# tangxyw/RecAlgorithm

Measured on NVIDIA H100. Metric: ctr_fwd_bwd_samples_per_sec, higher is better.
Workload: dtype f32

## Files before the change

### recalgorithm_b200/csrc/cin_bwd.cu

```cuda
#include <stdlib.h>

#include "tc_ptx.cuh"

namespace ctr {
namespace cinb {
using namespace ctr::tc;

__global__ void split_filter_native_kernel(const float* __restrict__ w, float* __restrict__ ws, int K, int H, int KRP, int HP) {
  const size_t total = (size_t)KRP * HP;
  for (size_t idx = (size_t)blockIdx.x * blockDim.x + threadIdx.x; idx < total; idx += (size_t)gridDim.x * blockDim.x) {
    const int row = (int)(idx / HP), n = (int)(idx % HP);
    float v = 0.f;
    if (row < K && n < H) v = __ldg(w + (size_t)row * H + n);
    store_split(ws, total, idx, v);
  }
}
__global__ void split_grad_kernel(const float* __restrict__ g, float* __restrict__ gs, size_t total) {
  for (size_t idx = (size_t)blockIdx.x * blockDim.x + threadIdx.x; idx < total; idx += (size_t)gridDim.x * blockDim.x)
    store_split(gs, total, idx, __ldg(g + idx));
}

constexpr int DX_IPS = 2;
constexpr int DX_N = DX_IPS * KB;
constexpr int DX_TILE = NWG * WG_M;

template <int SB, int NKB>
__global__ void __launch_bounds__(NTHREADS, 1)
cin_bwd_dx_tc_kernel(const __grid_constant__ CUtensorMap tmap_w, const float* __restrict__ x0,
                     const float* __restrict__ xk, const float* __restrict__ g, float* __restrict__ dx0,
                     float* __restrict__ dxk, int B, int m, int hk, int logD, int H, int KRP) {
  extern __shared__ __align__(1024) uint8_t smem_raw[];
  uint8_t* smem = align_1024(smem_raw);
  constexpr int HP = NKB * KB;
  constexpr int b_copy_bytes = NKB * DX_N * 128;
  constexpr int stage_bytes = 2 * b_copy_bytes;
  const uint32_t sbase = smem_u32(smem);
  Ring ring(sbase + SB * stage_bytes, SB);

  const int warp = warp_uniform(threadIdx.x >> 5), lane = threadIdx.x & 31;
  const int D = 1 << logD;
  const long long rows_total = (long long)B * D;
  const int num_tiles = (int)((rows_total + DX_TILE - 1) / DX_TILE);
  const int nsteps = (hk + DX_IPS - 1) / DX_IPS;

  ring.init();
  if (producer_role(warp, lane, [&] {
        for (int tile = blockIdx.x; tile < num_tiles; tile += gridDim.x) {
          for (int st = 0; st < nsteps; ++st) {
            const Ring::Slot slot = ring.acquire(stage_bytes);
            const uint32_t dst = sbase + slot.stage * stage_bytes;
            tma_load_4d(dst, &tmap_w, 0, st * DX_IPS * m, 0, 0, slot.full);
            tma_load_4d(dst + b_copy_bytes, &tmap_w, 0, KRP + st * DX_IPS * m, 0, 0, slot.full);
          }
        }
      }))
    return;

  const int wg = warp >> 2, w = warp & 3, gq = lane >> 2, t = lane & 3;
  for (int tile = blockIdx.x; tile < num_tiles; tile += gridDim.x) {
    const long long base = (long long)tile * DX_TILE + wg * WG_M;
    bool valid[2];
    int bb[2], dd[2];
    float x0v[2][8], dx0acc[2][8];
    uint32_t gh[HP / 8][4], gl[HP / 8][4];
#pragma unroll
    for (int rr = 0; rr < 2; ++rr) {
      const long long r = base + w * 16 + gq + 8 * rr;
      valid[rr] = r < rows_total;
      bb[rr] = valid[rr] ? (int)(r >> logD) : 0;
      dd[rr] = (int)(r & (D - 1));
#pragma unroll
      for (int q = 0; q < 8; ++q) {
        const int j = 8 * (q >> 1) + 2 * t + (q & 1);
        x0v[rr][q] = (valid[rr] && j < m) ? __ldg(x0 + ((size_t)bb[rr] * m + j) * D + dd[rr]) : 0.f;
        dx0acc[rr][q] = 0.f;
      }
    }
#pragma unroll
    for (int ks = 0; ks < HP / 8; ++ks) {
      float ga[4];
#pragma unroll
      for (int q = 0; q < 4; ++q) {
        const int rr = q & 1, n = 8 * ks + t + 4 * (q >> 1);
        ga[q] = (valid[rr] && n < H) ? __ldg(g + ((size_t)bb[rr] * H + n) * D + dd[rr]) : 0.f;
      }
      tf32_split(ga, gh[ks], gl[ks]);
    }
    auto load_xi = [&](int i0, float (&xi)[2][DX_IPS]) {
#pragma unroll
      for (int rr = 0; rr < 2; ++rr)
#pragma unroll
        for (int h = 0; h < DX_IPS; ++h)
          xi[rr][h] = (valid[rr] && i0 + h < hk) ? __ldg(xk + ((size_t)bb[rr] * hk + i0 + h) * D + dd[rr]) : 0.f;
    };
    float xi[2][DX_IPS];
    load_xi(0, xi);
    for (int st = 0; st < nsteps; ++st) {
      const int i0 = st * DX_IPS;
      const int s = ring.wait();
      const uint64_t bhi = gmma_desc_kmajor(sbase + s * stage_bytes, 128);
      const uint64_t blo = gmma_desc_kmajor(sbase + s * stage_bytes + b_copy_bytes, 128);
      float dz[DX_N / 2];
#pragma unroll
      for (int q = 0; q < DX_N / 2; ++q) dz[q] = 0.f;
      wgmma_fence();
#pragma unroll
      for (int ks = 0; ks < HP / 8; ++ks) {
        const uint64_t off = (uint64_t)((ks >> 2) * (DX_N * 128 / 16) + 2 * (ks & 3));
        mma_3xtf32<DX_N>(dz, gh[ks], gl[ks], bhi, blo, off, ks > 0 ? 1 : 0);
      }
      wgmma_commit();
      float xin[2][DX_IPS];
      load_xi(i0 + DX_IPS, xin);
      wgmma_wait<0>();
      ring.release(lane);
#pragma unroll
      for (int h = 0; h < DX_IPS; ++h) {
#pragma unroll
        for (int rr = 0; rr < 2; ++rr) {
          float p = 0.f;
#pragma unroll
          for (int q = 0; q < 8; ++q) {
            const float v = dz[4 * (4 * h + (q >> 1)) + 2 * rr + (q & 1)];
            p += v * x0v[rr][q];
            dx0acc[rr][q] += v * xi[rr][h];
          }
          p += __shfl_xor_sync(0xffffffffu, p, 1);
          p += __shfl_xor_sync(0xffffffffu, p, 2);
          if (t == 0 && valid[rr] && i0 + h < hk) dxk[((size_t)bb[rr] * hk + i0 + h) * D + dd[rr]] = p;
        }
      }
#pragma unroll
      for (int rr = 0; rr < 2; ++rr)
#pragma unroll
        for (int h = 0; h < DX_IPS; ++h) xi[rr][h] = xin[rr][h];
    }
#pragma unroll
    for (int rr = 0; rr < 2; ++rr) {
#pragma unroll
      for (int q = 0; q < 8; ++q) {
        const int j = 8 * (q >> 1) + 2 * t + (q & 1);
        if (valid[rr] && j < m) dx0[((size_t)bb[rr] * m + j) * D + dd[rr]] = dx0acc[rr][q];
      }
    }
  }
}

constexpr int DW_IPC = NWG * 2;

template <int N, int D>
__global__ void __launch_bounds__(NTHREADS, 1)
cin_bwd_dw_tc_kernel(const __grid_constant__ CUtensorMap tmap_g, const float* __restrict__ x0,
                     const float* __restrict__ xk, float* __restrict__ dw, int B, int m, int hk, int H,
                     int ngroups, int nslices, int chunk, int SB) {
  extern __shared__ __align__(1024) uint8_t smem_raw[];
  uint8_t* smem = align_1024(smem_raw);
  constexpr int row_bytes = D * 4;
  constexpr int b_copy_bytes = N * row_bytes;
  constexpr int stage_bytes = 2 * b_copy_bytes;
  const uint32_t sbase = smem_u32(smem);
  Ring ring(sbase + SB * stage_bytes, SB);

  const int warp = warp_uniform(threadIdx.x >> 5), lane = threadIdx.x & 31;
  const int group = blockIdx.x % ngroups;
  int b_beg, b_end;
  batch_slice(blockIdx.x / ngroups, nslices, B, b_beg, b_end);

  ring.init();
  if (producer_role(warp, lane, [&] {
        for (int b = b_beg; b < b_end; ++b) {
          const Ring::Slot slot = ring.acquire(stage_bytes);
          const uint32_t dst = sbase + slot.stage * stage_bytes;
          tma_load_3d(dst, &tmap_g, 0, 0, b, slot.full);
          tma_load_3d(dst + b_copy_bytes, &tmap_g, 0, 0, B + b, slot.full);
        }
      }))
    return;

  const int wg = warp >> 2, w = warp & 3, gq = lane >> 2, t = lane & 3;
  const int i = group * DW_IPC + wg * 2 + (w >> 1);
  const int j0 = (w & 1) * 16 + gq, j1 = j0 + 8;
  const bool live0 = i < hk && j0 < m, live1 = i < hk && j1 < m;
  float acc[N / 2], dacc[N / 2];
#pragma unroll
  for (int q = 0; q < N / 2; ++q) { acc[q] = 0.f; dacc[q] = 0.f; }
  auto form = [&](int b, uint32_t (&fh)[D / 8][4], uint32_t (&fl)[D / 8][4]) {
    float xa[D / 4], xb0[D / 4], xb1[D / 4];
#pragma unroll
    for (int q = 0; q < D / 4; ++q) {
      const int d = 8 * (q >> 1) + t + 4 * (q & 1);
      xa[q] = i < hk ? __ldg(xk + ((size_t)b * hk + i) * D + d) : 0.f;
      xb0[q] = live0 ? __ldg(x0 + ((size_t)b * m + j0) * D + d) : 0.f;
      xb1[q] = live1 ? __ldg(x0 + ((size_t)b * m + j1) * D + d) : 0.f;
    }
#pragma unroll
    for (int k = 0; k < D / 8; ++k) {
      const float a[4] = {xa[2 * k] * xb0[2 * k], xa[2 * k] * xb1[2 * k], xa[2 * k + 1] * xb0[2 * k + 1],
                          xa[2 * k + 1] * xb1[2 * k + 1]};
      tf32_split(a, fh[k], fl[k]);
    }
  };
  uint32_t ah[D / 8][4], al[D / 8][4];
  if (b_end > b_beg) form(b_beg, ah, al);
  for (int b = b_beg; b < b_end; ++b) {
    const bool chunk_start = chain_first(b - b_beg, chunk);
    const int s = ring.wait();
    const uint64_t bhi = gmma_desc_kmajor(sbase + s * stage_bytes, row_bytes);
    const uint64_t blo = gmma_desc_kmajor(sbase + s * stage_bytes + b_copy_bytes, row_bytes);
    wgmma_fence();
#pragma unroll
    for (int k = 0; k < D / 8; ++k) mma_3xtf32<N>(dacc, ah[k], al[k], bhi, blo, 2 * k, (chunk_start && k == 0) ? 0 : 1);
    wgmma_commit();
    uint32_t bh[D / 8][4], bl[D / 8][4];
    form(b + 1 < b_end ? b + 1 : b, bh, bl);
    wgmma_wait_keep(ah, al);
    ring.release(lane);
    if (chain_last(b - b_beg, b_end - b_beg, chunk)) chain_drain(acc, dacc);
#pragma unroll
    for (int k = 0; k < D / 8; ++k)
#pragma unroll
      for (int q = 0; q < 4; ++q) { ah[k][q] = bh[k][q]; al[k][q] = bl[k][q]; }
  }
  if (b_end > b_beg) {
#pragma unroll
    for (int c = 0; c < N / 8; ++c) {
#pragma unroll
      for (int e = 0; e < 2; ++e) {
        const int n = 8 * c + 2 * t + e;
        if (n < H) {
          if (live0) atomicAdd(dw + ((size_t)i * m + j0) * H + n, acc[4 * c + e]);
          if (live1) atomicAdd(dw + ((size_t)i * m + j1) * H + n, acc[4 * c + 2 + e]);
        }
      }
    }
  }
}

__global__ void __launch_bounds__(256)
cin_bwd_dx_kernel(const float* __restrict__ x0, const float* __restrict__ xk, const float* __restrict__ w,
                  const float* __restrict__ g, int B, int m, int hk, int D, int H, float* __restrict__ dx0,
                  float* __restrict__ dxk) {
  extern __shared__ __align__(16) float sm[];
  float* x0s = sm;
  float* xks = x0s + m * D;
  float* gs = xks + hk * D;
  float* dx0s = gs + H * D;
  float* dxks = dx0s + m * D;
  const int d = threadIdx.x % D, pl = threadIdx.x / D, pstep = blockDim.x / D;
  for (int b = blockIdx.x; b < B; b += gridDim.x) {
    __syncthreads();
    for (int i = threadIdx.x; i < m * D; i += blockDim.x) { x0s[i] = __ldg(x0 + (size_t)b * m * D + i); dx0s[i] = 0.f; }
    for (int i = threadIdx.x; i < hk * D; i += blockDim.x) { xks[i] = __ldg(xk + (size_t)b * hk * D + i); dxks[i] = 0.f; }
    for (int i = threadIdx.x; i < H * D; i += blockDim.x) gs[i] = __ldg(g + (size_t)b * H * D + i);
    __syncthreads();
    if (pl < pstep) {
      for (int p = pl; p < hk * m; p += pstep) {
        const float* wr = w + (size_t)p * H;
        float dz = 0.f;
        for (int n = 0; n < H; ++n) dz += gs[n * D + d] * __ldg(wr + n);
        const int i = p / m, j = p % m;
        atomicAdd(dxks + i * D + d, dz * x0s[j * D + d]);
        atomicAdd(dx0s + j * D + d, dz * xks[i * D + d]);
      }
    }
    __syncthreads();
    for (int i = threadIdx.x; i < m * D; i += blockDim.x) dx0[(size_t)b * m * D + i] = dx0s[i];
    for (int i = threadIdx.x; i < hk * D; i += blockDim.x) dxk[(size_t)b * hk * D + i] = dxks[i];
  }
}

constexpr int CIN_PC = 16;
__global__ void __launch_bounds__(256)
cin_bwd_dw_kernel(const float* __restrict__ x0, const float* __restrict__ xk, const float* __restrict__ g, int B, int m,
                  int hk, int D, int H, float* __restrict__ dw) {
  extern __shared__ __align__(16) float sm[];
  float* gs = sm;
  float* zs = gs + H * (D + 1);
  const int p0 = blockIdx.x * CIN_PC;
  const int K = hk * m;
  float acc[CIN_PC];
#pragma unroll
  for (int q = 0; q < CIN_PC; ++q) acc[q] = 0.f;
  for (int b = blockIdx.y; b < B; b += gridDim.y) {
    __syncthreads();
    for (int i = threadIdx.x; i < H * D; i += blockDim.x) gs[(i / D) * (D + 1) + i % D] = __ldg(g + (size_t)b * H * D + i);
    for (int i = threadIdx.x; i < CIN_PC * D; i += blockDim.x) {
      const int q = i / D, d = i % D, p = p0 + q;
      float z = 0.f;
      if (p < K) z = __ldg(xk + ((size_t)b * hk + p / m) * D + d) * __ldg(x0 + ((size_t)b * m + p % m) * D + d);
      zs[i] = z;
    }
    __syncthreads();
    for (int n = threadIdx.x; n < H; n += blockDim.x) {
      for (int d = 0; d < D; ++d) {
        const float gv = gs[n * (D + 1) + d];
#pragma unroll
        for (int q = 0; q < CIN_PC; ++q) acc[q] += zs[q * D + d] * gv;
      }
    }
  }
  const int n = threadIdx.x;
  if (n < H) {
#pragma unroll
    for (int q = 0; q < CIN_PC; ++q)
      if (p0 + q < K) atomicAdd(dw + (size_t)(p0 + q) * H + n, acc[q]);
  }
}

static bool tensor_path_ok(int64_t m, int64_t hk, int64_t D, int64_t H) {
  return m >= 1 && m <= 32 && hk >= 1 && H >= 1 && H <= 128 && (D == 8 || D == 16 || D == 32);
}

}
}

using namespace ctr;
using namespace ctr::cinb;

extern "C" int64_t ctr_cin_bwd_workspace_bytes(int64_t B, int64_t m, int64_t hk, int64_t D, int64_t H) {
  if (!tensor_path_ok(m, hk, D, H)) return 0;
  const int64_t HP = pad_to(H, 32), KRP = (hk + 2) * m + 32;
  return ((2 * KRP + m) * HP + 2 * B * H * D) * (int64_t)sizeof(float);
}

extern "C" int ctr_cin_bwd(const float* x0, const float* xk, const float* filter, const float* g_out, int64_t B,
                           int64_t m, int64_t hk, int64_t D, int64_t H, float* dx0, float* dxk, float* dfilter,
                           void* workspace, int64_t workspace_bytes, void* stream) {
  static const char* fn = "ctr_cin_bwd";
  CTR_REQUIRE(B >= 0 && m >= 1 && hk >= 1 && D >= 1 && H >= 1, "ctr_cin_bwd: bad sizes B=%lld m=%lld hk=%lld D=%lld H=%lld",
              (long long)B, (long long)m, (long long)hk, (long long)D, (long long)H);
  CTR_UNSUPPORTED(B * D > 0x7fffffffLL || hk * m > (1 << 24), "ctr_cin_bwd: problem too large");
  CTR_REQUIRE(x0 && xk && filter && g_out && dx0 && dxk && dfilter, "ctr_cin_bwd: null argument");
  CTR_UNSUPPORTED(D > 256 || H > 256, "ctr_cin_bwd: D=%lld H=%lld too large", (long long)D, (long long)H);
  cudaStream_t st = as_stream(stream);
  CTR_CUDA(cudaMemsetAsync(dfilter, 0, sizeof(float) * hk * m * H, st));
  if (B == 0) return CTR_OK;
  const int sms = sm_count();
  int rc;
  if (!tensor_path_ok(m, hk, D, H)) {
    const size_t smem_dx = sizeof(float) * (size_t)(2 * (m + hk) + H) * D;
    CTR_UNSUPPORTED(smem_dx > 200 * 1024, "ctr_cin_bwd: shared memory need %zu B too large", smem_dx);
    const int grid = capped_grid(B, (int64_t)sms * 4);
    rc = launch("ctr_cin_bwd(dx)", cin_bwd_dx_kernel, grid, 256, smem_dx, st, x0, xk, filter, g_out, (int)B, (int)m,
                (int)hk, (int)D, (int)H, dx0, dxk);
    if (rc) return rc;
    const size_t smem_dw = sizeof(float) * (size_t)(H * (D + 1) + CIN_PC * D);
    CTR_UNSUPPORTED(smem_dw > 200 * 1024, "ctr_cin_bwd: shared memory need %zu B too large", smem_dw);
    const int gx = (int)((hk * m + CIN_PC - 1) / CIN_PC);
    int gy = (int)((int64_t)sms * 4 / gx);
    if (gy < 1) gy = 1;
    if (gy > B) gy = (int)B;
    return launch("ctr_cin_bwd(dw)", cin_bwd_dw_kernel, dim3(gx, gy), 256, smem_dw, st, x0, xk, g_out, (int)B, (int)m,
                  (int)hk, (int)D, (int)H, dfilter);
  }
  rc = check_workspace(fn, "ctr_cin_bwd_workspace_bytes", workspace, workspace_bytes,
                       ctr_cin_bwd_workspace_bytes(B, m, hk, D, H));
  if (rc) return rc;
  const int HP = (int)pad_to(H, 32), KRP = (int)((hk + 2) * m + 32);
  const int NP = pad3(H);
  float* ws_w = static_cast<float*>(workspace);
  float* ws_g = ws_w + (size_t)(2 * KRP + m) * HP;
  rc = launch("ctr_cin_bwd(split filter)", split_filter_native_kernel, capped_grid(((size_t)KRP * HP + 255) / 256, 2048), 256, 0, st,
              filter, ws_w, (int)(hk * m), (int)H, KRP, HP);
  if (rc) return rc;
  const size_t tg = (size_t)B * H * D;
  rc = launch("ctr_cin_bwd(split grad)", split_grad_kernel, capped_grid((tg + 255) / 256, 4096), 256, 0, st, g_out, ws_g, tg);
  if (rc) return rc;
  int logD = 0;
  while ((1 << logD) < D) ++logD;
  {
    CUtensorMap tmap;
    const cuuint64_t gdim[4] = {32, (cuuint64_t)(2 * KRP), (cuuint64_t)DX_IPS, (cuuint64_t)(HP / 32)};
    const cuuint64_t gstr[3] = {(cuuint64_t)HP * sizeof(float), (cuuint64_t)m * HP * sizeof(float), 32 * sizeof(float)};
    const cuuint32_t box[4] = {32, 32, (cuuint32_t)DX_IPS, (cuuint32_t)(HP / 32)};
    rc = encode_tmap(fn, &tmap, 4, ws_w, gdim, gstr, box, CU_TENSOR_MAP_SWIZZLE_128B);
    if (rc) return rc;
    constexpr int SB = 3;
    const int nkb = HP / 32;
    const int smem = SB * 2 * nkb * DX_N * 128 + 8 * 2 * SB + 1024;
    const long long rows = (long long)B * D;
    const int tiles = (int)((rows + DX_TILE - 1) / DX_TILE);
    const int grid = capped_grid(tiles, sms);
    rc = with_const<1, 2, 3, 4>(nkb, [&](auto NKB) {
      return launch("ctr_cin_bwd(dx, wgmma)", cin_bwd_dx_tc_kernel<SB, NKB>, grid, NTHREADS, smem, st, tmap, x0, xk, g_out,
                    dx0, dxk, (int)B, (int)m, (int)hk, logD, (int)H, KRP);
    });
    if (rc) return rc;
  }
  CUtensorMap tmap;
  const cuuint64_t gdim[3] = {(cuuint64_t)D, (cuuint64_t)H, (cuuint64_t)(2 * B)};
  const cuuint64_t gstr[2] = {(cuuint64_t)D * sizeof(float), (cuuint64_t)H * D * sizeof(float)};
  const cuuint32_t box[3] = {(cuuint32_t)D, (cuuint32_t)NP, 1};
  const CUtensorMapSwizzle sw = D == 32 ? CU_TENSOR_MAP_SWIZZLE_128B : D == 16 ? CU_TENSOR_MAP_SWIZZLE_64B
                                                                               : CU_TENSOR_MAP_SWIZZLE_32B;
  rc = encode_tmap(fn, &tmap, 3, ws_g, gdim, gstr, box, sw);
  if (rc) return rc;
  const int stage_bytes = 2 * NP * (int)D * 4;
  int sb = (192 * 1024) / stage_bytes;
  if (sb > 8) sb = 8;
  const int smem = sb * stage_bytes + 8 * 2 * sb + 1024;
  const int ngroups = (int)((hk + DW_IPC - 1) / DW_IPC);
  const int nslices = batch_slices(sms, ngroups, B);
  const int grid = ngroups * nslices;
  const int chunk = (int)(256 / D);
  return with_const<32, 64, 128>(NP, [&](auto N) {
    return with_const<8, 16, 32>((int)D, [&](auto DD) {
      return launch("ctr_cin_bwd(dw, wgmma)", cin_bwd_dw_tc_kernel<N, DD>, grid, NTHREADS, smem, st, tmap, x0, xk,
                    dfilter, (int)B, (int)m, (int)hk, (int)H, ngroups, nslices, chunk, sb);
    });
  });
}
```

### recalgorithm_b200/csrc/tc_ptx.cuh

```cuda
#pragma once
#include <cuda.h>

#include "ctr_common.cuh"

namespace ctr {
namespace tc {

constexpr int WG_M = 64;
constexpr int KB = 32;
constexpr int NWG = 2;
constexpr int NTHREADS = (NWG + 1) * 128;

__device__ __forceinline__ uint32_t smem_u32(const void* p) { return (uint32_t)__cvta_generic_to_shared(p); }

__device__ __forceinline__ void mbar_init(uint32_t bar, uint32_t count) {
  asm volatile("mbarrier.init.shared::cta.b64 [%0], %1;" ::"r"(bar), "r"(count) : "memory");
}
__device__ __forceinline__ void mbar_arrive(uint32_t bar) {
  asm volatile("mbarrier.arrive.shared::cta.b64 _, [%0];" ::"r"(bar) : "memory");
}
__device__ __forceinline__ void mbar_expect_tx(uint32_t bar, uint32_t bytes) {
  asm volatile("mbarrier.arrive.expect_tx.shared::cta.b64 _, [%0], %1;" ::"r"(bar), "r"(bytes) : "memory");
}
__device__ __forceinline__ void mbar_wait(uint32_t bar, uint32_t parity) {
  asm volatile(
      "{\n"
      ".reg .pred p;\n"
      "WAIT_%=:\n"
      "mbarrier.try_wait.parity.shared::cta.b64 p, [%0], %1;\n"
      "@p bra DONE_%=;\n"
      "bra WAIT_%=;\n"
      "DONE_%=:\n"
      "}\n" ::"r"(bar), "r"(parity)
      : "memory");
}
__device__ __forceinline__ void fence_barrier_init() { asm volatile("fence.mbarrier_init.release.cluster;" ::: "memory"); }
__device__ __forceinline__ int warp_uniform(int v) { return __shfl_sync(0xffffffffu, v, 0); }
template <int R>
__device__ __forceinline__ void setmaxnreg_dec() { asm volatile("setmaxnreg.dec.sync.aligned.u32 %0;" ::"n"(R)); }
template <int R>
__device__ __forceinline__ void setmaxnreg_inc() { asm volatile("setmaxnreg.inc.sync.aligned.u32 %0;" ::"n"(R)); }
__device__ __forceinline__ void wg_bar_sync(int id) { asm volatile("bar.sync %0, 128;" ::"r"(id) : "memory"); }
__device__ __forceinline__ void consumers_bar() { asm volatile("bar.sync 1, 256;" ::: "memory"); }
__device__ __forceinline__ void fence_proxy_async() { asm volatile("fence.proxy.async.shared::cta;" ::: "memory"); }

__device__ __forceinline__ void tma_load_2d(uint32_t dst, const CUtensorMap* map, int c0, int c1, uint32_t bar) {
  asm volatile(
      "cp.async.bulk.tensor.2d.shared::cluster.global.tile.mbarrier::complete_tx::bytes [%0], [%1, {%2, %3}], [%4];"
      ::"r"(dst), "l"(map), "r"(c0), "r"(c1), "r"(bar)
      : "memory");
}
__device__ __forceinline__ void tma_load_3d(uint32_t dst, const CUtensorMap* map, int c0, int c1, int c2, uint32_t bar) {
  asm volatile(
      "cp.async.bulk.tensor.3d.shared::cluster.global.tile.mbarrier::complete_tx::bytes [%0], [%1, {%2, %3, %4}], [%5];"
      ::"r"(dst), "l"(map), "r"(c0), "r"(c1), "r"(c2), "r"(bar)
      : "memory");
}
__device__ __forceinline__ void tma_load_4d(uint32_t dst, const CUtensorMap* map, int c0, int c1, int c2, int c3, uint32_t bar) {
  asm volatile(
      "cp.async.bulk.tensor.4d.shared::cluster.global.tile.mbarrier::complete_tx::bytes [%0], [%1, {%2, %3, %4, %5}], [%6];"
      ::"r"(dst), "l"(map), "r"(c0), "r"(c1), "r"(c2), "r"(c3), "r"(bar)
      : "memory");
}

__device__ __forceinline__ float tf32_rna(float x) {
  uint32_t r;
  asm("cvt.rna.tf32.f32 %0, %1;" : "=r"(r) : "f"(x));
  return __uint_as_float(r);
}
__device__ __forceinline__ void tf32_split(const float (&a)[4], uint32_t (&hi)[4], uint32_t (&lo)[4]) {
#pragma unroll
  for (int q = 0; q < 4; ++q) {
    const float h = tf32_rna(a[q]);
    hi[q] = __float_as_uint(h);
    lo[q] = __float_as_uint(tf32_rna(a[q] - h));
  }
}

__device__ __forceinline__ uint64_t gmma_desc_kmajor(uint32_t saddr, int row_bytes) {
  uint64_t d = 0;
  d |= (uint64_t)((saddr & 0x3FFFF) >> 4);
  d |= (uint64_t)1 << 16;
  d |= (uint64_t)((8 * row_bytes) >> 4) << 32;
  d |= (uint64_t)(row_bytes == 128 ? 1 : row_bytes == 64 ? 2 : 3) << 62;
  return d;
}

__device__ __forceinline__ void wgmma_keep(uint32_t (&r)[4]) {
  asm volatile("" : "+r"(r[0]), "+r"(r[1]), "+r"(r[2]), "+r"(r[3])::"memory");
}
__device__ __forceinline__ void wgmma_fence() { asm volatile("wgmma.fence.sync.aligned;" ::: "memory"); }
__device__ __forceinline__ void wgmma_commit() { asm volatile("wgmma.commit_group.sync.aligned;" ::: "memory"); }
template <int N>
__device__ __forceinline__ void wgmma_wait() { asm volatile("wgmma.wait_group.sync.aligned %0;" ::"n"(N) : "memory"); }

template <int N>
__device__ __forceinline__ void wgmma_tf32_rs(float (&d)[N / 2], const uint32_t (&a)[4], uint64_t bdesc, int scale_d);
template <>
__device__ __forceinline__ void wgmma_tf32_rs<32>(float (&d)[16], const uint32_t (&a)[4], uint64_t bdesc, int scale_d) {
  asm volatile(
      "{\n.reg .pred p;\nsetp.ne.b32 p, %21, 0;\n"
      "wgmma.mma_async.sync.aligned.m64n32k8.f32.tf32.tf32 {%0,%1,%2,%3,%4,%5,%6,%7,%8,%9,%10,%11,%12,%13,%14,%15}, {%16,%17,%18,%19}, %20, p, 1, 1;\n}\n"
      : "+f"(d[0]), "+f"(d[1]), "+f"(d[2]), "+f"(d[3]), "+f"(d[4]), "+f"(d[5]), "+f"(d[6]), "+f"(d[7]), "+f"(d[8]), "+f"(d[9]), "+f"(d[10]), "+f"(d[11]), "+f"(d[12]), "+f"(d[13]), "+f"(d[14]), "+f"(d[15])
      : "r"(a[0]), "r"(a[1]), "r"(a[2]), "r"(a[3]), "l"(bdesc), "r"(scale_d));
}
template <>
__device__ __forceinline__ void wgmma_tf32_rs<64>(float (&d)[32], const uint32_t (&a)[4], uint64_t bdesc, int scale_d) {
  asm volatile(
      "{\n.reg .pred p;\nsetp.ne.b32 p, %37, 0;\n"
      "wgmma.mma_async.sync.aligned.m64n64k8.f32.tf32.tf32 {%0,%1,%2,%3,%4,%5,%6,%7,%8,%9,%10,%11,%12,%13,%14,%15,%16,%17,%18,%19,%20,%21,%22,%23,%24,%25,%26,%27,%28,%29,%30,%31}, {%32,%33,%34,%35}, %36, p, 1, 1;\n}\n"
      : "+f"(d[0]), "+f"(d[1]), "+f"(d[2]), "+f"(d[3]), "+f"(d[4]), "+f"(d[5]), "+f"(d[6]), "+f"(d[7]), "+f"(d[8]), "+f"(d[9]), "+f"(d[10]), "+f"(d[11]), "+f"(d[12]), "+f"(d[13]), "+f"(d[14]), "+f"(d[15]), "+f"(d[16]), "+f"(d[17]), "+f"(d[18]), "+f"(d[19]), "+f"(d[20]), "+f"(d[21]), "+f"(d[22]), "+f"(d[23]), "+f"(d[24]), "+f"(d[25]), "+f"(d[26]), "+f"(d[27]), "+f"(d[28]), "+f"(d[29]), "+f"(d[30]), "+f"(d[31])
      : "r"(a[0]), "r"(a[1]), "r"(a[2]), "r"(a[3]), "l"(bdesc), "r"(scale_d));
}
template <>
__device__ __forceinline__ void wgmma_tf32_rs<96>(float (&d)[48], const uint32_t (&a)[4], uint64_t bdesc, int scale_d) {
  asm volatile(
      "{\n.reg .pred p;\nsetp.ne.b32 p, %53, 0;\n"
      "wgmma.mma_async.sync.aligned.m64n96k8.f32.tf32.tf32 {%0,%1,%2,%3,%4,%5,%6,%7,%8,%9,%10,%11,%12,%13,%14,%15,%16,%17,%18,%19,%20,%21,%22,%23,%24,%25,%26,%27,%28,%29,%30,%31,%32,%33,%34,%35,%36,%37,%38,%39,%40,%41,%42,%43,%44,%45,%46,%47}, {%48,%49,%50,%51}, %52, p, 1, 1;\n}\n"
      : "+f"(d[0]), "+f"(d[1]), "+f"(d[2]), "+f"(d[3]), "+f"(d[4]), "+f"(d[5]), "+f"(d[6]), "+f"(d[7]), "+f"(d[8]), "+f"(d[9]), "+f"(d[10]), "+f"(d[11]), "+f"(d[12]), "+f"(d[13]), "+f"(d[14]), "+f"(d[15]), "+f"(d[16]), "+f"(d[17]), "+f"(d[18]), "+f"(d[19]), "+f"(d[20]), "+f"(d[21]), "+f"(d[22]), "+f"(d[23]), "+f"(d[24]), "+f"(d[25]), "+f"(d[26]), "+f"(d[27]), "+f"(d[28]), "+f"(d[29]), "+f"(d[30]), "+f"(d[31]), "+f"(d[32]), "+f"(d[33]), "+f"(d[34]), "+f"(d[35]), "+f"(d[36]), "+f"(d[37]), "+f"(d[38]), "+f"(d[39]), "+f"(d[40]), "+f"(d[41]), "+f"(d[42]), "+f"(d[43]), "+f"(d[44]), "+f"(d[45]), "+f"(d[46]), "+f"(d[47])
      : "r"(a[0]), "r"(a[1]), "r"(a[2]), "r"(a[3]), "l"(bdesc), "r"(scale_d));
}
template <>
__device__ __forceinline__ void wgmma_tf32_rs<128>(float (&d)[64], const uint32_t (&a)[4], uint64_t bdesc, int scale_d) {
  asm volatile(
      "{\n.reg .pred p;\nsetp.ne.b32 p, %69, 0;\n"
      "wgmma.mma_async.sync.aligned.m64n128k8.f32.tf32.tf32 {%0,%1,%2,%3,%4,%5,%6,%7,%8,%9,%10,%11,%12,%13,%14,%15,%16,%17,%18,%19,%20,%21,%22,%23,%24,%25,%26,%27,%28,%29,%30,%31,%32,%33,%34,%35,%36,%37,%38,%39,%40,%41,%42,%43,%44,%45,%46,%47,%48,%49,%50,%51,%52,%53,%54,%55,%56,%57,%58,%59,%60,%61,%62,%63}, {%64,%65,%66,%67}, %68, p, 1, 1;\n}\n"
      : "+f"(d[0]), "+f"(d[1]), "+f"(d[2]), "+f"(d[3]), "+f"(d[4]), "+f"(d[5]), "+f"(d[6]), "+f"(d[7]), "+f"(d[8]), "+f"(d[9]), "+f"(d[10]), "+f"(d[11]), "+f"(d[12]), "+f"(d[13]), "+f"(d[14]), "+f"(d[15]), "+f"(d[16]), "+f"(d[17]), "+f"(d[18]), "+f"(d[19]), "+f"(d[20]), "+f"(d[21]), "+f"(d[22]), "+f"(d[23]), "+f"(d[24]), "+f"(d[25]), "+f"(d[26]), "+f"(d[27]), "+f"(d[28]), "+f"(d[29]), "+f"(d[30]), "+f"(d[31]), "+f"(d[32]), "+f"(d[33]), "+f"(d[34]), "+f"(d[35]), "+f"(d[36]), "+f"(d[37]), "+f"(d[38]), "+f"(d[39]), "+f"(d[40]), "+f"(d[41]), "+f"(d[42]), "+f"(d[43]), "+f"(d[44]), "+f"(d[45]), "+f"(d[46]), "+f"(d[47]), "+f"(d[48]), "+f"(d[49]), "+f"(d[50]), "+f"(d[51]), "+f"(d[52]), "+f"(d[53]), "+f"(d[54]), "+f"(d[55]), "+f"(d[56]), "+f"(d[57]), "+f"(d[58]), "+f"(d[59]), "+f"(d[60]), "+f"(d[61]), "+f"(d[62]), "+f"(d[63])
      : "r"(a[0]), "r"(a[1]), "r"(a[2]), "r"(a[3]), "l"(bdesc), "r"(scale_d));
}

template <int N>
__device__ __forceinline__ void mma_3xtf32(float (&d)[N / 2], const uint32_t (&ah)[4], const uint32_t (&al)[4], uint64_t bhi,
                                           uint64_t blo, uint64_t off, int scale_d) {
  wgmma_tf32_rs<N>(d, al, bhi + off, scale_d);
  wgmma_tf32_rs<N>(d, ah, blo + off, 1);
  wgmma_tf32_rs<N>(d, ah, bhi + off, 1);
}
template <int NK>
__device__ __forceinline__ void wgmma_wait_keep(uint32_t (&ah)[NK][4], uint32_t (&al)[NK][4]) {
  wgmma_wait<0>();
#pragma unroll
  for (int k = 0; k < NK; ++k) { wgmma_keep(ah[k]); wgmma_keep(al[k]); }
}

__device__ __forceinline__ bool chain_first(int i, int len) { return i % len == 0; }
__device__ __forceinline__ bool chain_last(int i, int n, int len) { return (i + 1) % len == 0 || i + 1 == n; }
template <int N>
__device__ __forceinline__ void chain_drain(float (&acc)[N], const float (&dacc)[N]) {
#pragma unroll
  for (int q = 0; q < N; ++q) acc[q] += dacc[q];
}

__device__ __forceinline__ void store_split(float* dst, size_t total, size_t idx, float v) {
  const float hi = tf32_rna(v);
  dst[idx] = hi;
  dst[total + idx] = v - hi;
}
__device__ __forceinline__ void store_split_sw128(float* tile, int rows, int k, int b, float v) {
  const uint32_t o = (uint32_t)(k * 128 + b * 4);
  store_split(tile, rows * 32, (o ^ (((o >> 7) & 7u) << 4)) / 4, v);
}

__device__ __forceinline__ uint8_t* align_1024(uint8_t* smem_raw) {
  return smem_raw + ((1024u - (smem_u32(smem_raw) & 1023u)) & 1023u);
}

struct Ring {
  uint32_t bar0;
  int nstages;
  int s = 0;
  uint32_t ph = 0;

  __device__ __forceinline__ Ring(uint32_t bar0_, int nstages_) : bar0(bar0_), nstages(nstages_) {}
  __device__ __forceinline__ uint32_t full() const { return bar0 + 8 * s; }
  __device__ __forceinline__ uint32_t empty() const { return bar0 + 8 * (nstages + s); }
  __device__ __forceinline__ void advance() {
    if (++s == nstages) { s = 0; ph ^= 1; }
  }
  __device__ __forceinline__ void init() const {
    if (threadIdx.x == 0) {
      for (int i = 0; i < nstages; ++i) { mbar_init(bar0 + 8 * i, 1); mbar_init(bar0 + 8 * (nstages + i), NWG * 4); }
      fence_barrier_init();
    }
    __syncthreads();
  }
  struct Slot {
    int stage;
    uint32_t full;
  };
  __device__ __forceinline__ Slot acquire(uint32_t bytes) {
    mbar_wait(empty(), ph ^ 1);
    mbar_expect_tx(full(), bytes);
    const Slot slot = {s, full()};
    advance();
    return slot;
  }
  __device__ __forceinline__ int wait() const {
    mbar_wait(full(), ph);
    return s;
  }
  __device__ __forceinline__ void release(int lane) {
    if (lane == 0) mbar_arrive(empty());
    advance();
  }
};

template <class Producer>
__device__ __forceinline__ bool producer_role(int warp, int lane, Producer&& producer) {
  if (warp >= NWG * 4) {
    setmaxnreg_dec<40>();
    if (warp == NWG * 4 && lane == 0) producer();
    return true;
  }
  setmaxnreg_inc<232>();
  return false;
}

__device__ __forceinline__ void batch_slice(int slice, int nslices, int n_units, int& beg, int& end) {
  const int per_slice = (n_units + nslices - 1) / nslices;
  beg = min(n_units, slice * per_slice);
  end = min(n_units, beg + per_slice);
}

constexpr int DW_BC = KB;
constexpr int DW_NC = NWG * WG_M;

template <int N, class Stage, class QOf, class POf>
__device__ __forceinline__ void batch_reduce(float (&acc)[N / 2], Ring& ring, uint8_t* qts, int c_beg, int c_end, int B,
                                             int lane, int nl0, Stage&& stage_chunk, QOf&& q_of, POf&& p_of) {
  constexpr int qt_bytes = 2 * N * 128;
  constexpr int CHAIN = 8;
  const int t = lane & 3;
  float dacc[N / 2];
#pragma unroll
  for (int q = 0; q < N / 2; ++q) { acc[q] = 0.f; dacc[q] = 0.f; }
  for (int c = c_beg; c < c_end; ++c) {
    const int b0 = c * DW_BC;
    stage_chunk(b0);
    const int s = ring.wait();
    float* qt = reinterpret_cast<float*>(qts + s * qt_bytes);
    for (int idx = threadIdx.x; idx < N * DW_BC; idx += NWG * 128) {
      const int k = idx / DW_BC, b = idx % DW_BC;
      store_split_sw128(qt, N, k, b, b0 + b < B ? q_of(k, b0, b) : 0.f);
    }
    fence_proxy_async();
    consumers_bar();
    uint32_t ah[4][4], al[4][4];
#pragma unroll
    for (int ks = 0; ks < 4; ++ks) {
      float a[4];
#pragma unroll
      for (int q = 0; q < 4; ++q) a[q] = p_of(s, 8 * ks + t + 4 * (q >> 1), nl0 + 8 * (q & 1));
      tf32_split(a, ah[ks], al[ks]);
    }
    const bool chain_start = chain_first(c - c_beg, CHAIN);
    const uint64_t bhi = gmma_desc_kmajor(smem_u32(qt), 128);
    const uint64_t blo = gmma_desc_kmajor(smem_u32(qt + N * 32), 128);
    wgmma_fence();
#pragma unroll
    for (int ks = 0; ks < 4; ++ks) mma_3xtf32<N>(dacc, ah[ks], al[ks], bhi, blo, 2 * ks, (chain_start && ks == 0) ? 0 : 1);
    wgmma_commit();
    wgmma_wait_keep(ah, al);
    ring.release(lane);
    if (chain_last(c - c_beg, c_end - c_beg, CHAIN)) chain_drain(acc, dacc);
  }
}

struct GradRow {
  float* dst = nullptr;
  int stride = 0;
  float* bias = nullptr;
};

__device__ __forceinline__ void red_add_global(float* p, float v) {
  asm volatile("red.global.add.f32 [%0], %1;" ::"l"(__cvta_generic_to_global(p)), "f"(v) : "memory");
}

__host__ __device__ constexpr int dw_smem_bytes(int N, int SB) { return SB * (2 * N * 128 + DW_BC * DW_NC * 4 + 16); }

template <int N, class Rows>
__global__ void __launch_bounds__(NTHREADS, 1)
weight_grad_wgmma_kernel(const __grid_constant__ CUtensorMap tmap_p, const float* __restrict__ q,
                         const float* __restrict__ qmask, const Rows rows, int rows_total, int d, int ngroups, int nslices,
                         int SB) {
  extern __shared__ __align__(1024) uint8_t smem_raw[];
// ... 147 lines not shown

template <int NW>
__device__ __forceinline__ void load_ks_stage(uint32_t dst, const CUtensorMap* map, int u0, int kb, int NP, uint32_t bar) {
  tma_load_2d(dst, map, kb * KB, u0, bar);
  tma_load_2d(dst + 2 * NW * 128, map, kb * KB, NP + u0, bar);
}

template <int NW>
__device__ __forceinline__ void gemm_ks(float (&d)[NW / 2], const float* xs, int ldx, int nk, int r0, int t, int lane,
                                        int wg, Ring& ring, uint32_t sbase) {
  float dacc[NW / 2];
#pragma unroll
  for (int q = 0; q < NW / 2; ++q) { d[q] = 0.f; dacc[q] = 0.f; }
  for (int kb = 0; kb < nk; ++kb) {
    const uint32_t st = sbase + ring.wait() * ks_stage_bytes<NW>() + wg * NW * 128;
    const uint64_t bhi = gmma_desc_kmajor(st, 128), blo = gmma_desc_kmajor(st + 2 * NW * 128, 128);
    uint32_t ah[4][4], al[4][4];
#pragma unroll
    for (int ks = 0; ks < 4; ++ks) {
      float a[4];
#pragma unroll
      for (int q = 0; q < 4; ++q) a[q] = xs[(r0 + 8 * (q & 1)) * ldx + kb * KB + 8 * ks + t + 4 * (q >> 1)];
      tf32_split(a, ah[ks], al[ks]);
    }
    wgmma_fence();
#pragma unroll
    for (int ks = 0; ks < 4; ++ks) mma_3xtf32<NW>(dacc, ah[ks], al[ks], bhi, blo, (uint64_t)(2 * ks), ks == 0 ? 0 : 1);
    wgmma_commit();
    wgmma_wait_keep(ah, al);
    ring.release(lane);
    chain_drain(d, dacc);
  }
}

}

constexpr size_t SMEM_CAP = 226 * 1024;

static inline int64_t pad_to(int64_t v, int64_t q) { return (v + q - 1) / q * q; }
static inline int pad3(int64_t v) { return v <= 32 ? 32 : v <= 64 ? 64 : 128; }
static inline int check_workspace(const char* fn, const char* size_fn, const void* ws, int64_t bytes, int64_t need) {
  CTR_REQUIRE(ws != nullptr && bytes >= need, "%s: workspace of %lld bytes required (%s), got %lld", fn, (long long)need,
              size_fn, (long long)bytes);
  CTR_REQUIRE((reinterpret_cast<uintptr_t>(ws) & 127) == 0, "%s: workspace must be 128-byte aligned", fn);
  return CTR_OK;
}

static inline int encode_tmap(const char* fn, CUtensorMap* map, int rank, const void* base, const cuuint64_t* dims,
                              const cuuint64_t* byte_strides, const cuuint32_t* box, CUtensorMapSwizzle swizzle) {
  typedef CUresult (*EncodeTiledFn)(CUtensorMap*, CUtensorMapDataType, cuuint32_t, void*, const cuuint64_t*,
                                    const cuuint64_t*, const cuuint32_t*, const cuuint32_t*, CUtensorMapInterleave,
                                    CUtensorMapSwizzle, CUtensorMapL2promotion, CUtensorMapFloatOOBfill);
  static EncodeTiledFn enc = nullptr;
  if (enc == nullptr) {
    void* p = nullptr;
    cudaDriverEntryPointQueryResult q;
    if (cudaGetDriverEntryPoint("cuTensorMapEncodeTiled", &p, cudaEnableDefault, &q) == cudaSuccess &&
        q == cudaDriverEntryPointSuccess)
      enc = reinterpret_cast<EncodeTiledFn>(p);
  }
  if (enc == nullptr) {
    set_error("%s: cuTensorMapEncodeTiled is not available from the driver", fn);
    return CTR_ERR_CUDA;
  }
  const cuuint32_t elem_strides[5] = {1, 1, 1, 1, 1};
  CUresult cr = enc(map, CU_TENSOR_MAP_DATA_TYPE_FLOAT32, rank, const_cast<void*>(base), dims, byte_strides, box,
                    elem_strides, CU_TENSOR_MAP_INTERLEAVE_NONE, swizzle, CU_TENSOR_MAP_L2_PROMOTION_L2_256B,
                    CU_TENSOR_MAP_FLOAT_OOB_FILL_NONE);
  if (cr != CUDA_SUCCESS) {
    set_error("%s: cuTensorMapEncodeTiled failed with CUresult %d", fn, (int)cr);
    return CTR_ERR_CUDA;
  }
  return CTR_OK;
}

static inline int encode_2d(const char* fn, CUtensorMap* map, const void* base, uint64_t inner, uint64_t outer,
                            uint32_t box_inner, uint32_t box_outer, CUtensorMapSwizzle sw) {
  const cuuint64_t gdim[2] = {(cuuint64_t)inner, (cuuint64_t)outer};
  const cuuint64_t gstr[1] = {(cuuint64_t)inner * sizeof(float)};
  const cuuint32_t box[2] = {box_inner, box_outer};
  return encode_tmap(fn, map, 2, base, gdim, gstr, box, sw);
}

static inline int batch_slices(int sms, int64_t ngroups, int64_t n_units) {
  int64_t n = sms / ngroups;
  if (n < 1) n = 1;
  return (int)(n < n_units ? n : n_units);
}
static inline int stages_that_fit(size_t fixed, size_t stage) {
  const size_t sb = (SMEM_CAP - fixed) / stage;
  return (int)(sb < 4 ? sb : 4);
}
template <int N, class Rows>
static inline int launch_weight_grad(const char* fn, const char* what, const Rows& rows, const float* p, int64_t units,
                                     int64_t rows_total, const float* q, const float* qmask, int d, int n_ds,
                                     cudaStream_t st) {
  CUtensorMap map;
  if (int rc = encode_2d(fn, &map, p, units, rows_total, DW_NC, DW_BC, CU_TENSOR_MAP_SWIZZLE_NONE)) return rc;
  const int ngroups = (int)((units + DW_NC - 1) / DW_NC);
  const int nslices = batch_slices(sm_count() / n_ds, ngroups, (rows_total + DW_BC - 1) / DW_BC);
  const int sb = stages_that_fit(1024, dw_smem_bytes(N, 1));
  return launch(what, weight_grad_wgmma_kernel<N, Rows>, dim3(ngroups * nslices, n_ds), NTHREADS, dw_smem_bytes(N, sb) + 1024,
                st, map, q, qmask, rows, (int)rows_total, d, ngroups, nslices, sb);
}

namespace rows {
static inline int encode_rows_operand(const char* fn, CUtensorMap* map, const float* base, int DP, int64_t R) {
  return encode_2d(fn, map, base, DP, 2 * R, KB, HC, CU_TENSOR_MAP_SWIZZLE_128B);
}
static inline int encode_hidden_operand(const char* fn, CUtensorMap* map, const float* base, int DP, int64_t R) {
  return encode_2d(fn, map, base, R, 2 * DP, KB, DP, CU_TENSOR_MAP_SWIZZLE_128B);
}
static inline int dp_class(int64_t d) { return d <= 32 ? 32 : d <= 64 ? 64 : d <= 96 ? 96 : 128; }
}

}
}
```

Baseline: 111.8 million.

## Run CIN backward GEMM kernels as CTA pairs with TMA multicast operand loads

Both CIN backward tensor-core kernels now launch as 2-CTA clusters. Each CTA loads half of the shared hi/lo operand stage and multicasts it to both CTAs, and empty barriers are released across the pair. The dw kernel also groups several batch samples per stage (a 32-wide K dimension), which lengthens the MMA chain per barrier round and changes the chunk size. This aims to halve the L2/TMA traffic per CTA and cut per-stage synchronization. In exchange it adds cluster-wide barriers, couples paired CTAs' progress, and needs padded group counts.

```diff
diff --git a/recalgorithm_b200/csrc/cin_bwd.cu b/recalgorithm_b200/csrc/cin_bwd.cu
--- a/recalgorithm_b200/csrc/cin_bwd.cu
+++ b/recalgorithm_b200/csrc/cin_bwd.cu
@@ -43,22 +43,25 @@
   const int num_tiles = (int)((rows_total + DX_TILE - 1) / DX_TILE);
   const int nsteps = (hk + DX_IPS - 1) / DX_IPS;
 
-  ring.init();
+  const int rank = cluster_rank();
+  const int npairs = (num_tiles + 1) / 2, pair0 = blockIdx.x / 2, pair_step = gridDim.x / 2;
+  ring.init_pair();
   if (producer_role(warp, lane, [&] {
-        for (int tile = blockIdx.x; tile < num_tiles; tile += gridDim.x) {
+        for (int pair = pair0; pair < npairs; pair += pair_step) {
           for (int st = 0; st < nsteps; ++st) {
             const Ring::Slot slot = ring.acquire(stage_bytes);
-            const uint32_t dst = sbase + slot.stage * stage_bytes;
-            tma_load_4d(dst, &tmap_w, 0, st * DX_IPS * m, 0, 0, slot.full);
-            tma_load_4d(dst + b_copy_bytes, &tmap_w, 0, KRP + st * DX_IPS * m, 0, 0, slot.full);
+            tma_load_4d_pair(sbase + slot.stage * stage_bytes + rank * b_copy_bytes, &tmap_w, 0, rank * KRP + st * DX_IPS * m,
+                             0, 0, slot.full);
           }
         }
-      }))
+      })) {
+    cluster_sync();
     return;
+  }
 
   const int wg = warp >> 2, w = warp & 3, gq = lane >> 2, t = lane & 3;
-  for (int tile = blockIdx.x; tile < num_tiles; tile += gridDim.x) {
-    const long long base = (long long)tile * DX_TILE + wg * WG_M;
+  for (int pair = pair0; pair < npairs; pair += pair_step) {
+    const long long base = (long long)(2 * pair + rank) * DX_TILE + wg * WG_M;
     bool valid[2];
     int bb[2], dd[2];
     float x0v[2][8], dx0acc[2][8];
@@ -113,7 +116,7 @@
       float xin[2][DX_IPS];
       load_xi(i0 + DX_IPS, xin);
       wgmma_wait<0>();
-      ring.release(lane);
+      ring.release_pair(lane);
 #pragma unroll
       for (int h = 0; h < DX_IPS; ++h) {
 #pragma unroll
@@ -144,9 +147,11 @@
       }
     }
   }
+  cluster_sync();
 }
 
 constexpr int DW_IPC = NWG * 2;
+constexpr int DW_SD = 32;
 
 template <int N, int D>
 __global__ void __launch_bounds__(NTHREADS, 1)
@@ -155,27 +160,31 @@
                      int ngroups, int nslices, int chunk, int SB) {
   extern __shared__ __align__(1024) uint8_t smem_raw[];
   uint8_t* smem = align_1024(smem_raw);
+  constexpr int S = DW_SD / D;
+  constexpr int NK = S * (D / 8);
   constexpr int row_bytes = D * 4;
-  constexpr int b_copy_bytes = N * row_bytes;
+  constexpr int tile_bytes = N * row_bytes;
+  constexpr int b_copy_bytes = S * tile_bytes;
   constexpr int stage_bytes = 2 * b_copy_bytes;
   const uint32_t sbase = smem_u32(smem);
   Ring ring(sbase + SB * stage_bytes, SB);
 
   const int warp = warp_uniform(threadIdx.x >> 5), lane = threadIdx.x & 31;
   const int group = blockIdx.x % ngroups;
-  int b_beg, b_end;
-  batch_slice(blockIdx.x / ngroups, nslices, B, b_beg, b_end);
-
-  ring.init();
+  int u_beg, u_end;
+  batch_slice(blockIdx.x / ngroups, nslices, (B + S - 1) / S, u_beg, u_end);
+
+  const int rank = cluster_rank();
+  ring.init_pair();
   if (producer_role(warp, lane, [&] {
-        for (int b = b_beg; b < b_end; ++b) {
+        for (int u = u_beg; u < u_end; ++u) {
           const Ring::Slot slot = ring.acquire(stage_bytes);
-          const uint32_t dst = sbase + slot.stage * stage_bytes;
-          tma_load_3d(dst, &tmap_g, 0, 0, b, slot.full);
-          tma_load_3d(dst + b_copy_bytes, &tmap_g, 0, 0, B + b, slot.full);
+          tma_load_4d_pair(sbase + slot.stage * stage_bytes + rank * b_copy_bytes, &tmap_g, 0, 0, u * S, rank, slot.full);
         }
-      }))
+      })) {
+    cluster_sync();
     return;
+  }
 
   const int wg = warp >> 2, w = warp & 3, gq = lane >> 2, t = lane & 3;
   const int i = group * DW_IPC + wg * 2 + (w >> 1);
@@ -184,44 +193,53 @@
   float acc[N / 2], dacc[N / 2];
 #pragma unroll
   for (int q = 0; q < N / 2; ++q) { acc[q] = 0.f; dacc[q] = 0.f; }
-  auto form = [&](int b, uint32_t (&fh)[D / 8][4], uint32_t (&fl)[D / 8][4]) {
-    float xa[D / 4], xb0[D / 4], xb1[D / 4];
-#pragma unroll
-    for (int q = 0; q < D / 4; ++q) {
-      const int d = 8 * (q >> 1) + t + 4 * (q & 1);
-      xa[q] = i < hk ? __ldg(xk + ((size_t)b * hk + i) * D + d) : 0.f;
-      xb0[q] = live0 ? __ldg(x0 + ((size_t)b * m + j0) * D + d) : 0.f;
-      xb1[q] = live1 ? __ldg(x0 + ((size_t)b * m + j1) * D + d) : 0.f;
-    }
-#pragma unroll
-    for (int k = 0; k < D / 8; ++k) {
-      const float a[4] = {xa[2 * k] * xb0[2 * k], xa[2 * k] * xb1[2 * k], xa[2 * k + 1] * xb0[2 * k + 1],
-                          xa[2 * k + 1] * xb1[2 * k + 1]};
-      tf32_split(a, fh[k], fl[k]);
+  float xa[S][D / 4], xb0[S][D / 4], xb1[S][D / 4];
+  auto load = [&](int u) {
+#pragma unroll
+    for (int s = 0; s < S; ++s) {
+      const int b = u * S + s;
+      const bool ok = u < u_end && b < B;
+#pragma unroll
+      for (int q = 0; q < D / 4; ++q) {
+        const int d = 8 * (q >> 1) + t + 4 * (q & 1);
+        xa[s][q] = ok && i < hk ? __ldg(xk + ((size_t)b * hk + i) * D + d) : 0.f;
+        xb0[s][q] = ok && live0 ? __ldg(x0 + ((size_t)b * m + j0) * D + d) : 0.f;
+        xb1[s][q] = ok && live1 ? __ldg(x0 + ((size_t)b * m + j1) * D + d) : 0.f;
+      }
     }
   };
-  uint32_t ah[D / 8][4], al[D / 8][4];
-  if (b_end > b_beg) form(b_beg, ah, al);
-  for (int b = b_beg; b < b_end; ++b) {
-    const bool chunk_start = chain_first(b - b_beg, chunk);
-    const int s = ring.wait();
-    const uint64_t bhi = gmma_desc_kmajor(sbase + s * stage_bytes, row_bytes);
-    const uint64_t blo = gmma_desc_kmajor(sbase + s * stage_bytes + b_copy_bytes, row_bytes);
+  uint32_t ah[NK][4], al[NK][4];
+  auto form = [&] {
+#pragma unroll
+    for (int s = 0; s < S; ++s)
+#pragma unroll
+      for (int k = 0; k < D / 8; ++k) {
+        const float a[4] = {xa[s][2 * k] * xb0[s][2 * k], xa[s][2 * k] * xb1[s][2 * k],
+                            xa[s][2 * k + 1] * xb0[s][2 * k + 1], xa[s][2 * k + 1] * xb1[s][2 * k + 1]};
+        tf32_split(a, ah[s * (D / 8) + k], al[s * (D / 8) + k]);
+      }
+  };
+  load(u_beg);
+  form();
+  for (int u = u_beg; u < u_end; ++u) {
+    const bool chunk_start = chain_first(u - u_beg, chunk);
+    const int st = ring.wait();
+    const uint64_t bhi = gmma_desc_kmajor(sbase + st * stage_bytes, row_bytes);
+    const uint64_t blo = gmma_desc_kmajor(sbase + st * stage_bytes + b_copy_bytes, row_bytes);
     wgmma_fence();
 #pragma unroll
-    for (int k = 0; k < D / 8; ++k) mma_3xtf32<N>(dacc, ah[k], al[k], bhi, blo, 2 * k, (chunk_start && k == 0) ? 0 : 1);
+    for (int kk = 0; kk < NK; ++kk) {
+      const uint64_t off = (uint64_t)((kk / (D / 8)) * (tile_bytes / 16) + 2 * (kk % (D / 8)));
+      mma_3xtf32<N>(dacc, ah[kk], al[kk], bhi, blo, off, (chunk_start && kk == 0) ? 0 : 1);
+    }
     wgmma_commit();
-    uint32_t bh[D / 8][4], bl[D / 8][4];
-    form(b + 1 < b_end ? b + 1 : b, bh, bl);
+    load(u + 1);
     wgmma_wait_keep(ah, al);
-    ring.release(lane);
-    if (chain_last(b - b_beg, b_end - b_beg, chunk)) chain_drain(acc, dacc);
-#pragma unroll
-    for (int k = 0; k < D / 8; ++k)
-#pragma unroll
-      for (int q = 0; q < 4; ++q) { ah[k][q] = bh[k][q]; al[k][q] = bl[k][q]; }
-  }
-  if (b_end > b_beg) {
+    ring.release_pair(lane);
+    if (chain_last(u - u_beg, u_end - u_beg, chunk)) chain_drain(acc, dacc);
+    form();
+  }
+  if (u_end > u_beg) {
 #pragma unroll
     for (int c = 0; c < N / 8; ++c) {
 #pragma unroll
@@ -234,6 +252,7 @@
       }
     }
   }
+  cluster_sync();
 }
 
 __global__ void __launch_bounds__(256)
@@ -380,33 +399,36 @@
     const int smem = SB * 2 * nkb * DX_N * 128 + 8 * 2 * SB + 1024;
     const long long rows = (long long)B * D;
     const int tiles = (int)((rows + DX_TILE - 1) / DX_TILE);
-    const int grid = capped_grid(tiles, sms);
     rc = with_const<1, 2, 3, 4>(nkb, [&](auto NKB) {
-      return launch("ctr_cin_bwd(dx, wgmma)", cin_bwd_dx_tc_kernel<SB, NKB>, grid, NTHREADS, smem, st, tmap, x0, xk, g_out,
-                    dx0, dxk, (int)B, (int)m, (int)hk, logD, (int)H, KRP);
+      const int cap = pair_capacity(cin_bwd_dx_tc_kernel<SB, NKB>, smem);
+      const int grid = 2 * capped_grid((tiles + 1) / 2, cap > 0 ? cap : sms / 2);
+      return launch_pairs("ctr_cin_bwd(dx, wgmma)", cin_bwd_dx_tc_kernel<SB, NKB>, grid, smem, st, tmap, x0, xk, g_out,
+                          dx0, dxk, (int)B, (int)m, (int)hk, logD, (int)H, KRP);
     });
     if (rc) return rc;
   }
+  const int S = DW_SD / (int)D;
   CUtensorMap tmap;
-  const cuuint64_t gdim[3] = {(cuuint64_t)D, (cuuint64_t)H, (cuuint64_t)(2 * B)};
-  const cuuint64_t gstr[2] = {(cuuint64_t)D * sizeof(float), (cuuint64_t)H * D * sizeof(float)};
-  const cuuint32_t box[3] = {(cuuint32_t)D, (cuuint32_t)NP, 1};
+  const cuuint64_t gdim[4] = {(cuuint64_t)D, (cuuint64_t)H, (cuuint64_t)B, 2};
+  const cuuint64_t gstr[3] = {(cuuint64_t)D * sizeof(float), (cuuint64_t)H * D * sizeof(float), (cuuint64_t)tg * sizeof(float)};
+  const cuuint32_t box[4] = {(cuuint32_t)D, (cuuint32_t)NP, (cuuint32_t)S, 1};
   const CUtensorMapSwizzle sw = D == 32 ? CU_TENSOR_MAP_SWIZZLE_128B : D == 16 ? CU_TENSOR_MAP_SWIZZLE_64B
                                                                                : CU_TENSOR_MAP_SWIZZLE_32B;
-  rc = encode_tmap(fn, &tmap, 3, ws_g, gdim, gstr, box, sw);
+  rc = encode_tmap(fn, &tmap, 4, ws_g, gdim, gstr, box, sw);
   if (rc) return rc;
-  const int stage_bytes = 2 * NP * (int)D * 4;
+  const int stage_bytes = 2 * NP * DW_SD * 4;
   int sb = (192 * 1024) / stage_bytes;
   if (sb > 8) sb = 8;
   const int smem = sb * stage_bytes + 8 * 2 * sb + 1024;
-  const int ngroups = (int)((hk + DW_IPC - 1) / DW_IPC);
-  const int nslices = batch_slices(sms, ngroups, B);
-  const int grid = ngroups * nslices;
-  const int chunk = (int)(256 / D);
+  const int ngroups = (int)pad_to((hk + DW_IPC - 1) / DW_IPC, 2);
+  const int units = (int)((B + S - 1) / S);
+  const int chunk = 8;
   return with_const<32, 64, 128>(NP, [&](auto N) {
     return with_const<8, 16, 32>((int)D, [&](auto DD) {
-      return launch("ctr_cin_bwd(dw, wgmma)", cin_bwd_dw_tc_kernel<N, DD>, grid, NTHREADS, smem, st, tmap, x0, xk,
-                    dfilter, (int)B, (int)m, (int)hk, (int)H, ngroups, nslices, chunk, sb);
+      const int cap = pair_capacity(cin_bwd_dw_tc_kernel<N, DD>, smem);
+      const int nslices = batch_slices(cap > 0 ? 2 * cap : sms, ngroups, units);
+      return launch_pairs("ctr_cin_bwd(dw, wgmma)", cin_bwd_dw_tc_kernel<N, DD>, ngroups * nslices, smem, st, tmap, x0,
+                          xk, dfilter, (int)B, (int)m, (int)hk, (int)H, ngroups, nslices, chunk, sb);
     });
   });
 }
diff --git a/recalgorithm_b200/csrc/tc_ptx.cuh b/recalgorithm_b200/csrc/tc_ptx.cuh
--- a/recalgorithm_b200/csrc/tc_ptx.cuh
+++ b/recalgorithm_b200/csrc/tc_ptx.cuh
@@ -60,6 +60,37 @@
   asm volatile(
       "cp.async.bulk.tensor.4d.shared::cluster.global.tile.mbarrier::complete_tx::bytes [%0], [%1, {%2, %3, %4, %5}], [%6];"
       ::"r"(dst), "l"(map), "r"(c0), "r"(c1), "r"(c2), "r"(c3), "r"(bar)
+      : "memory");
+}
+
+__device__ __forceinline__ int cluster_rank() {
+  uint32_t r;
+  asm volatile("mov.u32 %0, %%cluster_ctarank;" : "=r"(r));
+  return (int)r;
+}
+__device__ __forceinline__ void cluster_sync() {
+  __syncwarp();
+  asm volatile("barrier.cluster.arrive.release.aligned;\nbarrier.cluster.wait.acquire.aligned;" ::: "memory");
+}
+__device__ __forceinline__ void mbar_arrive_cta(uint32_t bar, int cta) {
+  asm volatile(
+      "{\n.reg .b32 ra;\nmapa.shared::cluster.u32 ra, %0, %1;\nmbarrier.arrive.release.cluster.shared::cluster.b64 _, [ra];\n}"
+      ::"r"(bar), "r"(cta)
+      : "memory");
+}
+__device__ __forceinline__ void tma_load_3d_pair(uint32_t dst, const CUtensorMap* map, int c0, int c1, int c2, uint32_t bar) {
+  asm volatile(
+      "cp.async.bulk.tensor.3d.shared::cluster.global.tile.mbarrier::complete_tx::bytes.multicast::cluster"
+      " [%0], [%1, {%2, %3, %4}], [%5], %6;"
+      ::"r"(dst), "l"(map), "r"(c0), "r"(c1), "r"(c2), "r"(bar), "h"((uint16_t)3)
+      : "memory");
+}
+__device__ __forceinline__ void tma_load_4d_pair(uint32_t dst, const CUtensorMap* map, int c0, int c1, int c2, int c3,
+                                                 uint32_t bar) {
+  asm volatile(
+      "cp.async.bulk.tensor.4d.shared::cluster.global.tile.mbarrier::complete_tx::bytes.multicast::cluster"
+      " [%0], [%1, {%2, %3, %4, %5}], [%6], %7;"
+      ::"r"(dst), "l"(map), "r"(c0), "r"(c1), "r"(c2), "r"(c3), "r"(bar), "h"((uint16_t)3)
       : "memory");
 }
 
@@ -201,6 +232,18 @@
   }
   __device__ __forceinline__ void release(int lane) {
     if (lane == 0) mbar_arrive(empty());
+    advance();
+  }
+
+  __device__ __forceinline__ void init_pair() const {
+    if (threadIdx.x == 0) {
+      for (int i = 0; i < nstages; ++i) { mbar_init(bar0 + 8 * i, 1); mbar_init(bar0 + 8 * (nstages + i), 2 * NWG * 4); }
+      fence_barrier_init();
+    }
+    cluster_sync();
+  }
+  __device__ __forceinline__ void release_pair(int lane) {
+    if (lane < 2) mbar_arrive_cta(empty(), lane);
     advance();
   }
 };
@@ -514,6 +557,39 @@
   return encode_tmap(fn, map, 2, base, gdim, gstr, box, sw);
 }
 
+static inline cudaLaunchConfig_t pair_config(cudaLaunchAttribute* attr, int grid, size_t smem, cudaStream_t st) {
+  attr->id = cudaLaunchAttributeClusterDimension;
+  attr->val.clusterDim.x = 2;
+  attr->val.clusterDim.y = 1;
+  attr->val.clusterDim.z = 1;
+  cudaLaunchConfig_t cfg = {};
+  cfg.gridDim = dim3(grid);
+  cfg.blockDim = dim3(NTHREADS);
+  cfg.dynamicSmemBytes = smem;
+  cfg.stream = st;
+  cfg.attrs = attr;
+  cfg.numAttrs = 1;
+  return cfg;
+}
+template <class... P>
+static inline int pair_capacity(void (*k)(P...), size_t smem) {
+  if (cudaFuncSetAttribute(k, cudaFuncAttributeMaxDynamicSharedMemorySize, (int)smem) != cudaSuccess) return 0;
+  cudaLaunchAttribute attr;
+  const cudaLaunchConfig_t cfg = pair_config(&attr, 2, smem, 0);
+  int n = 0;
+  if (cudaOccupancyMaxActiveClusters(&n, k, &cfg) != cudaSuccess) n = 0;
+  return n;
+}
+template <class... P, class... A>
+static inline int launch_pairs(const char* what, void (*k)(P...), int grid, size_t smem, cudaStream_t st, const A&... args) {
+  CTR_CUDA(cudaFuncSetAttribute(k, cudaFuncAttributeMaxDynamicSharedMemorySize, (int)smem));
+  cudaLaunchAttribute attr;
+  const cudaLaunchConfig_t cfg = pair_config(&attr, grid, smem, st);
+  CTR_CUDA(cudaLaunchKernelEx(&cfg, k, static_cast<P>(args)...));
+  CTR_CHECK_LAUNCH(what);
+  return CTR_OK;
+}
+
 static inline int batch_slices(int sms, int64_t ngroups, int64_t n_units) {
   int64_t n = sms / ngroups;
   if (n < 1) n = 1;
```

Result: no change. 111.7 million, median of 6 (-0.1%).
